# vqdang/hover_net

Hardware: NVIDIA B200
Metric: tiles/sec (higher is better)
Workload: dtype f16x3-split (fp32-equivalent products, fp32 accumulate); post-proc int32/f64

## Files before the change

### hover_net_b200/csrc/api.cu

```cuda
#include <cstring>
#include <memory>
#include <string>

#include "../../include/hvn.h"
#include "cnn.h"
#include "postproc.h"
#include "tile.h"

using namespace hvn;

static thread_local std::string g_err;

struct hvn_ctx {
    int device = 0;
    cudaStream_t stream = nullptr;
    std::unique_ptr<Model> model;
    Arena pp_arena;
    Arena io_arena;
    Arena tile_arena;
    int chunk = 0;
    int profile = 0;
    cudaEvent_t ev[4] = {nullptr, nullptr, nullptr, nullptr};
    cudaEvent_t tev[2] = {nullptr, nullptr};
    float ms_cnn = 0.f, ms_pp = 0.f;
// ... 94 lines not shown
    HVN_CHECK(c->model, HVN_ERR_STATE, "context has no model");
    c->model->finalize();
    API_END
}

int hvn_set_option(hvn_ctx *c, const char *key, int64_t value) {
    API_BEGIN
    use(c);
    std::string k = key ? key : "";
    if (k == "conv_path") { HVN_CHECK(c->model, HVN_ERR_STATE, "context has no model"); c->model->conv_path = (int)value; }
    else if (k == "chunk") c->chunk = (int)value;
    else if (k == "flood_impl") postproc_set_flood_impl((int)value);
    else if (k == "fuse_up2") { HVN_CHECK(c->model, HVN_ERR_STATE, "context has no model"); c->model->fuse_up2 = (int)value; }
    else if (k == "fuse_shortcut") { HVN_CHECK(c->model, HVN_ERR_STATE, "context has no model"); c->model->fuse_shortcut = (int)value; }
    else if (k == "stem_tc") { HVN_CHECK(c->model, HVN_ERR_STATE, "context has no model"); c->model->stem_tc = (int)value; }
    else if (k == "xform") { HVN_CHECK(c->model, HVN_ERR_STATE, "context has no model"); c->model->xform = (int)value; }
    else if (k == "branch_streams") { HVN_CHECK(c->model, HVN_ERR_STATE, "context has no model"); c->model->branch_streams = (int)value; }
    else if (k == "tc_seg_chunks") tc_set_seg_chunks((int)value);
    else if (k == "tc_block_n") tc_set_block_n((int)value);
    else if (k == "tc_res_tma") tc_set_res_tma((int)value);
    else if (k == "tc_xf_trunc") tc_set_xf_trunc((int)value);
    else if (k == "tc_ar") tc_set_ar((int)value);
    else if (k == "tc_lean_epi") tc_set_lean_epi((int)value);
    else if (k == "tc_rowstack") tc_set_rowstack((int)value);
    else if (k == "tc_xf_early") tc_set_xf_early((int)value);
    else if (k == "tc_prefetch") tc_set_prefetch((int)value);
    else if (k == "tc_ar_min_chunks") tc_set_ar_min_chunks((int)value);
    else if (k == "tc_ar_nres") tc_set_ar_nres((int)value);
    else if (k == "tc_ar_min_wst") tc_set_ar_min_wst((int)value);
    else if (k == "tc_res_tma_max_chunks") tc_set_res_tma_max_chunks((int)value);
// ... 411 lines not shown
```

### hover_net_b200/csrc/cnn.cu

```cuda
#include "cnn.h"

#include <algorithm>
#include <cmath>
#include <cstring>

namespace hvn {

static const struct { const char *name; int cin, c1, c3, units, stride; } kGroups[4] = {
    {"d0", 64, 64, 256, 3, 1}, {"d1", 256, 128, 512, 4, 2}, {"d2", 512, 256, 1024, 6, 2}, {"d3", 1024, 512, 2048, 3, 2}};

Plan::~Plan() {
    for (void *p : allocs) cudaFree(p);
}

template <typename T> T *Model::dalloc(size_t n, std::vector<void *> &owner, bool zero) {
    T *p = nullptr;
    HVN_CUDA(cudaMalloc((void **)&p, std::max<size_t>(n, 1) * sizeof(T)));
    owner.push_back(p);
    if (zero) HVN_CUDA(cudaMemset(p, 0, std::max<size_t>(n, 1) * sizeof(T)));
    return p;
}

void Model::add_spec(const std::string &name, std::initializer_list<int64_t> shape, bool ignored) {
    ParamSpec s;
// ... 393 lines not shown
    v.hi += off; v.lo += off; v.h = h; v.w = w; v.c = c;
    return v;
}
RawRef rview(const RawRef &b, int y0, int x0, int h, int w, int c0, int c) {
    RawRef v = b;
    v.p += (long long)y0 * b.sH + (long long)x0 * b.sW + c0;
    v.h = h; v.w = w; v.c = c;
    return v;
}
}

Plan &Model::plan(int B, int H, int W) {
    HVN_CHECK(finalized, -5, "weights not finalised (call hvn_finalize_weights)");
    HVN_CHECK(H == W, -1, "only square patches are supported (reference patch geometry is square)");
    std::string key = std::to_string(B) + "x" + std::to_string(H) + "x" + std::to_string(W) + "p" + std::to_string(conv_path) +
                      "b" + std::to_string(branch_streams) + "x" + std::to_string(xform) + "f" + std::to_string(fuse_shortcut) + "u" + std::to_string(fuse_up2) + "h" + std::to_string(tc_halo);
    auto it = plans_.find(key);
    if (it != plans_.end()) return *it->second;
    std::unique_ptr<Plan> pl(new Plan());
    Plan &P = *pl;
    P.B = B; P.H = H; P.W = W;
    out_shape(H, W, P.oh, P.ow, P.oc);

    auto new_split = [&](int h, int w, int c) {
        SplitRef r;
        size_t n = (size_t)B * h * w * c;
        r.hi = dalloc<__half>(n, P.allocs, true);
        r.lo = dalloc<__half>(n, P.allocs, true);
        P.bytes += 2 * n * sizeof(__half);
        r.sN = (long long)h * w * c; r.sH = w * c; r.sW = c; r.h = h; r.w = w; r.c = c;
        r.flag = d_flag_;
// ... 56 lines not shown
        op.c0_out = X0; op.c0_pad = mode == "fast" ? 3 : 0;
        op.bn = bn_.at("conv0.bn");
        op.flops = 2.0 * B * s0 * s0 * 64 * 147;
        P.ops.push_back(op);
    }
    SplitRef x = X0, D[4];
    int si = s0, ds[4];
    for (int gi = 0; gi < 4; ++gi) {
        const auto &g = kGroups[gi];
        const std::string gn = g.name;
        int so = (si + g.stride - 1) / g.stride;
        RawRef S = new_raw(so, so, g.c3);
        SplitRef A1 = new_split(si, si, g.c1), A2 = new_split(so, so, g.c1), Pp = new_split(so, so, g.c3);
        const bool fuse = fuse_shortcut != 0;
        if (!fuse) { Op &op = add_conv(gn + ".shortcut.weight", x, g.stride, 0, so, so); op.cp.out_raw = S; }
        for (int u = 0; u < g.units; ++u) {
            std::string p = gn + ".units." + std::to_string(u) + ".";
            const SplitRef &in = u == 0 ? x : Pp;
            int ri = u == 0 ? si : so, st = u == 0 ? g.stride : 1;
            SplitRef a1 = A1;
            if (ri != A1.h) { a1.h = ri; a1.w = ri; a1.sH = ri * g.c1; a1.sN = (long long)ri * ri * g.c1; }
            {
                Op &op = add_conv(p + "conv1.weight", in, 1, 0, ri, ri);
                set_bn(op, p + "conv1/bn", a1);
                if (u != 0 && use_xf) {
                    const BNParams &pb = bn_.at(p + "preact/bn");
                    op.cp.a_raw = S; op.cp.in_scale = pb.scale; op.cp.in_shift = pb.shift;
                }
            }
            int lo = tf_same_lo(ri, 3, st);
            { Op &op = add_conv(p + "conv2.weight", a1, st, lo, so, so); set_bn(op, p + "conv2/bn", A2); }
            {
                Op &op = add_conv(p + "conv3.weight", A2, 1, 0, so, so);
                if (u == 0 && fuse) {
                    op.cp.w = conv_.at(gn + ".fused3");
                    op.cp.a2 = x; op.cp.a2_stride = g.stride; op.cp.cin1 = g.c1;
                    op.flops += 2.0 * B * so * so * (double)g.cin * g.c3;
                    op.name = gn + ".units.0.conv3+shortcut";
                } else op.cp.res = S;
                if (u + 1 < g.units) {
                    op.cp.out_raw = S;
                    if (!use_xf) set_bn(op, gn + ".units." + std::to_string(u + 1) + ".preact/bn", Pp);
                } else set_bn(op, gn + ".blk_bna.bn", Pp);
            }
        }
        x = Pp; D[gi] = Pp; ds[gi] = so; si = so;
    }
    HVN_CHECK(2 * ds[3] == ds[2] && 2 * ds[2] == ds[1] && 2 * ds[1] == ds[0], -1, "patch size breaks the skip geometry");
    auto crop_to = [&](const SplitRef &d, int t) {
        int c = d.h - t;
        HVN_CHECK(c >= 0, -1, "skip connection smaller than decoder tensor");
        return sview(d, c / 2, c / 2, t, t, 0, d.c);
    };
    SplitRef U3in = new_split(2 * ds[3], 2 * ds[3], 1024);
    if (fuse_up2) {
        Op &op = add_conv("conv_bot.weight", D[3], 1, 0, ds[3], ds[3]);
        op.cp.up2 = 1; op.cp.skip = crop_to(D[2], 2 * ds[3]); op.cp.out_split = U3in;
    } else {
// ... 67 lines not shown
        if (b == 0) P.ops[first_op].fork_point = true;
        head.head.feat[b] = Hf[b];
        head.head.w[b] = head_w_.at(bp + "u0.conv");
        head.head.bias[b] = head_b_.at(bp + "u0.conv");
        head.head.out_ch[b] = branches_[b] == "tp" ? nr_types : 2;
        head.head.kind[b] = branches_[b] == "tp" ? HEAD_TP : (branches_[b] == "np" ? HEAD_NP : HEAD_HV);
        head.flops += 2.0 * B * ho * ho * 64 * head.head.out_ch[b];
    }
    cur_stream = 0;
    P.ops.push_back(head);

    tc_set_halo(tc_halo);
    for (auto &op : P.ops) {
        P.flops += op.flops;
        if (op.kind == Op::CONV && conv_path != 1) tc_plan(op.cp, op.tc);
    }
    plans_[key] = std::move(pl);
    return *plans_[key];
}

void Model::forward(const uint8_t *imgs, int B, int H, int W, float *out, int chunk, cudaStream_t s) {
    HVN_CHECK(finalized, -5, "weights not finalised (call hvn_finalize_weights)");
    HVN_CHECK(B >= 1, -1, "empty batch");
    int oh, ow, oc;
    out_shape(H, W, oh, ow, oc);
    if (chunk <= 0) chunk = 32;
    if (!side_[0]) {
        for (auto &st : side_) HVN_CUDA(cudaStreamCreateWithFlags(&st, cudaStreamNonBlocking));
        HVN_CUDA(cudaEventCreateWithFlags(&ev_fork_, cudaEventDisableTiming));
        for (auto &e : ev_join_) HVN_CUDA(cudaEventCreateWithFlags(&e, cudaEventDisableTiming));
// ... 43 lines not shown
                r.cls = "conv0";
                break;
            case Op::CONV:
                if (op.tc.ok && conv_path == 2) selftest_conv(op, s);
                if (op.tc.ok) { tc_launch(op.cp, op.tc, s); ++tc_launches; r.cls = "conv_tc"; }
                else {
                    ConvParams q = op.cp;
                    if (q.in_scale) {
                        launch_bnrelu(q.a_raw, bc, q.in_scale, q.in_shift, q.a, s);
                        q.in_scale = q.in_shift = nullptr;
                    }
                    launch_conv_ref(q, s);
                    r.cls = "conv_ref";
                }
                break;
            case Op::BNRELU:
                launch_bnrelu(op.bn_in, bc, op.bn.scale, op.bn.shift, op.bn_out, s);
                r.cls = "bnrelu";
                break;
            case Op::UP2ADD:
                launch_up2_add(op.up_in, bc, op.up_skip, op.up_out, s);
                r.cls = "bnrelu";
                break;
            case Op::HEAD: {
                HeadParams hp = op.head;
                hp.out = out + (size_t)b0 * oh * ow * oc;
                launch_head(hp, s);
                r.cls = "head";
                break;
            }
// ... 2 lines not shown
            if (profile_ops) { HVN_CUDA(cudaEventRecord(r.b, s)); recs.push_back(r); }
        }
    }
    s = main_stream;
    HVN_CUDA(cudaMemcpyAsync(h_flag_, d_flag_, sizeof(unsigned int), cudaMemcpyDeviceToHost, s));
    HVN_CUDA(cudaGetLastError());
    if (profile_ops) {
        HVN_CUDA(cudaStreamSynchronize(s));
        for (auto &r : recs) {
            float ms = 0.f;
            HVN_CUDA(cudaEventElapsedTime(&ms, r.a, r.b));
            class_ms[r.cls] += ms; class_flops[r.cls] += r.flops; class_launches[r.cls] += 1;
            if (profile_ops >= 2) {
                char line[384];
                const Op &o = *r.op;
                if (o.kind == Op::CONV)
                    snprintf(line, sizeof(line), "%-44s %-8s k%dx%d s%d cin%-4d cout%-4d out%dx%d box=%dx%d%s bn=%d %8.4f ms %8.2f GFLOP %7.1f TFLOP/s\n",
                             o.name.c_str(), r.cls, o.cp.w.kh, o.cp.w.kw, o.cp.stride, o.cp.w.cin, o.cp.w.cout, o.cp.ho, o.cp.wo,
                             o.tc.bw, o.tc.bh, o.tc.halo ? "H" : "", o.tc.block_n, ms, r.flops / 1e9, r.flops / 1e9 / std::max(ms, 1e-6f));
                else
                    snprintf(line, sizeof(line), "%-44s %-8s %8.4f ms\n", o.name.c_str(), r.cls, ms);
                debug_log += line;
            }
            cudaEventDestroy(r.a); cudaEventDestroy(r.b);
        }
    }
}

}
```

### hover_net_b200/csrc/cnn.h

```cpp
#pragma once
#include <map>
#include <memory>
#include <string>
#include <vector>

#include "cnn_kernels.h"
#include "common.cuh"

namespace hvn {

struct ParamSpec {
    std::string name;
    int ndim = 0;
    int64_t shape[4] = {0, 0, 0, 0};
    bool ignored = false;
    bool loaded = false;
    size_t numel() const {
        size_t n = 1;
        for (int i = 0; i < ndim; ++i) n *= (size_t)shape[i];
        return n;
    }
};

struct BNParams { float *scale = nullptr, *shift = nullptr; int c = 0; };

struct Op {
    enum Kind { CONV0, CONV, BNRELU, HEAD, UP2ADD } kind = CONV;
    std::string name;
    ConvParams cp;
    TcPlan tc;
    SplitRef c0_out; int c0_pad = 0;
    RawRef bn_in; SplitRef bn_out; BNParams bn;
    HeadParams head;
    RawRef up_in; SplitRef up_skip, up_out;
    double flops = 0;
    int stream = 0;
    bool fork_point = false;
};

struct Plan {
    int B = 0, H = 0, W = 0, oh = 0, ow = 0, oc = 0;
    std::vector<Op> ops;
    std::vector<void *> allocs;
    size_t bytes = 0;
    double flops = 0;
// ... 4 lines not shown
  public:
    Model(const std::string &mode, int nr_types);
    ~Model();
    std::string mode;
    int nr_types;
    int k;
    std::vector<ParamSpec> spec;
    std::map<std::string, int> index;
    std::map<std::string, std::vector<float>> host;
    bool finalized = false;
    int tc_halo = 1;
    int fuse_up2 = 0;
    int fuse_shortcut = 1;
    int stem_tc = 1;
    int xform = 1;
    int branch_streams = 1;
    int conv_path = 0;
    int act_shift = 0;
    bool range_overflow() const { return h_flag_ && *h_flag_ != 0; }
    void reset_range_flag(cudaStream_t s);

    void load(const std::string &name, const float *data, int ndim, const int64_t *shape);
    void finalize();
    void out_shape(int H, int W, int &oh, int &ow, int &oc) const;
    Plan &plan(int B, int H, int W);
    void forward(const uint8_t *imgs, int B, int H, int W, float *out, int chunk, cudaStream_t s);

    long long kernel_launches = 0, tc_launches = 0;
    int profile_ops = 0;
    std::map<std::string, double> class_ms, class_flops;
// ... 29 lines not shown
```

### hover_net_b200/csrc/cnn_kernels.h

```cpp
#pragma once
#include <cuda_runtime.h>
#include "conv_params.h"

#define HVN_MAX_TYPES 16

namespace hvn {

enum HeadKind { HEAD_TP = 0, HEAD_NP = 1, HEAD_HV = 2 };

struct HeadParams {
    int nbranch = 0;
    SplitRef feat[3];
    const float *w[3] = {nullptr, nullptr, nullptr};
    const float *bias[3] = {nullptr, nullptr, nullptr};
    int out_ch[3] = {0, 0, 0};
    int kind[3] = {0, 0, 0};
    int B = 0, h = 0, w_ = 0, C = 0;
    float *out = nullptr;
};

void launch_conv_ref(const ConvParams &P, cudaStream_t s);
void launch_conv0(const uint8_t *img, int B, int H, int W, int pad, const float *wgt, const float *scale,
                  const float *shift, const SplitRef &out, cudaStream_t s);
bool conv0_tc_supported(int H, int W, int pad, const SplitRef &out);
// ... 9 lines not shown
    unsigned char tmap_a_hi[128], tmap_a_lo[128], tmap_w_hi[128], tmap_w_lo[128];
    unsigned char tmap_a2_hi[128], tmap_a2_lo[128];
    int bw = 0, bh = 0;
    int tiles_x = 0, tiles_y = 0;
    int block_n = 0;
    int flat = 0;
    int res_tma = 0;
    int rs = 0, rs_bw = 0, rs_bh = 0;
    unsigned char tmap_rs_w_hi[128], tmap_rs_w_lo[128];
    int ar = 0, ar_gn = 1;
    int halo = 0;
    int halo_w = 0, halo_h = 0;
};
bool tc_plan(const ConvParams &P, TcPlan &plan);
void tc_launch(const ConvParams &P, const TcPlan &plan, cudaStream_t s);
void tc_set_block_n(int n);
void tc_set_seg_chunks(int n);
void tc_set_res_tma(int on);
void tc_set_res_tma_max_chunks(int n);
void tc_set_ar(int on);
void tc_set_ar_min_chunks(int n);
void tc_set_ar_nres(int n);
void tc_set_ar_min_wst(int n);
void tc_set_prefetch(int n);
void tc_set_rowstack(int on);
void tc_set_lean_epi(int on);
void tc_set_xf_early(int on);
void tc_set_xf_trunc(int on);
void tc_set_halo(int mode);

// ... 2 lines not shown
```

### hover_net_b200/csrc/conv_tc.cu

```cuda
#include <cuda.h>
#include <cuda_runtime.h>

#include <mutex>

#include "common.cuh"
#include "conv_epilogue.cuh"
#include "cnn_kernels.h"

namespace hvn {

__device__ __forceinline__ uint32_t smem_u32(const void *p) { return (uint32_t)__cvta_generic_to_shared(p); }

__device__ __forceinline__ void mbar_init(uint32_t bar, uint32_t count) {
    asm volatile("mbarrier.init.shared::cta.b64 [%0], %1;" ::"r"(bar), "r"(count) : "memory");
}
__device__ __forceinline__ void mbar_expect_tx(uint32_t bar, uint32_t bytes) {
    asm volatile("mbarrier.arrive.expect_tx.shared::cta.b64 _, [%0], %1;" ::"r"(bar), "r"(bytes) : "memory");
}
__device__ __forceinline__ void mbar_arrive(uint32_t bar) {
    asm volatile("mbarrier.arrive.shared::cta.b64 _, [%0];" ::"r"(bar) : "memory");
}
__device__ __forceinline__ void mbar_wait(uint32_t bar, uint32_t parity) {
    uint32_t ok;
    do {
// ... 28 lines not shown
    asm volatile(
        "{\n\t.reg .pred p;\n\t"
        "setp.ne.b32 p, %4, 0;\n\t"
        "tcgen05.mma.cta_group::1.kind::f16 [%0], %1, %2, %3, p;\n\t}"
        ::"r"(tmem_d), "l"(adesc), "l"(bdesc), "r"(idesc), "r"(accum) : "memory");
}
__device__ __forceinline__ void tc_ld32(uint32_t taddr, uint32_t (&r)[32]) {
    asm volatile(
        "tcgen05.ld.sync.aligned.32x32b.x32.b32 "
        "{%0, %1, %2, %3, %4, %5, %6, %7, %8, %9, %10, %11, %12, %13, %14, %15, "
        "%16, %17, %18, %19, %20, %21, %22, %23, %24, %25, %26, %27, %28, %29, %30, %31}, [%32];"
        : "=r"(r[0]), "=r"(r[1]), "=r"(r[2]), "=r"(r[3]), "=r"(r[4]), "=r"(r[5]), "=r"(r[6]), "=r"(r[7]),
          "=r"(r[8]), "=r"(r[9]), "=r"(r[10]), "=r"(r[11]), "=r"(r[12]), "=r"(r[13]), "=r"(r[14]), "=r"(r[15]),
          "=r"(r[16]), "=r"(r[17]), "=r"(r[18]), "=r"(r[19]), "=r"(r[20]), "=r"(r[21]), "=r"(r[22]), "=r"(r[23]),
          "=r"(r[24]), "=r"(r[25]), "=r"(r[26]), "=r"(r[27]), "=r"(r[28]), "=r"(r[29]), "=r"(r[30]), "=r"(r[31])
        : "r"(taddr) : "memory");
}
__device__ __forceinline__ void tc_ld_wait() { asm volatile("tcgen05.wait::ld.sync.aligned;" ::: "memory"); }

__device__ __forceinline__ uint64_t umma_desc(uint32_t saddr, uint32_t sbo = 1024) {
    uint64_t d = 0;
    d |= (uint64_t)((saddr & 0x3FFFFu) >> 4);
    d |= (uint64_t)1 << 16;
    d |= (uint64_t)(sbo >> 4) << 32;
    d |= (uint64_t)1 << 46;
    d |= (uint64_t)2 << 61;
    return d;
}

struct TcGeom {
// ... 726 lines not shown
                }
                asm volatile("fence.proxy.async.shared::cta;" ::: "memory");
                __syncwarp();
                if (lane == 0) request_res(tc + G.nres);
            }
        }
    }
    tc_fence_before();
    __syncthreads();
    if (warp == 1) {
        tc_fence_after();
        asm volatile("tcgen05.dealloc.cta_group::1.sync.aligned.b32 %0, %1;" ::"r"(tmem_base), "r"(TMEM_COLS) : "memory");
    }
}

struct RsGeom {
    int bw, bh, rows, tiles_y, tiles_m, kchunks, kh, seg;
};
template <int KW> constexpr int rs_stages() { return KW >= 5 ? 2 : 3; }
template <int KW> constexpr int rs_max_rows() { return KW >= 5 ? 124 : 128; }
template <int KW> constexpr int rs_stage_bytes() { return 2 * A_TILE_BYTES + 2 * KW * 32 * 128; }
template <int KW> constexpr int rs_smem() {
    return 1024 + rs_stages<KW>() * rs_stage_bytes<KW>() + 2 * rs_max_rows<KW>() * (KW * 16 + 4) * 4 + 8 * (2 * rs_stages<KW>() + 4) + 16;
}

__device__ __forceinline__ void tc_ld16(uint32_t taddr, uint32_t (&r)[16]) {
    asm volatile(
        "tcgen05.ld.sync.aligned.32x32b.x16.b32 "
        "{%0, %1, %2, %3, %4, %5, %6, %7, %8, %9, %10, %11, %12, %13, %14, %15}, [%16];"
        : "=r"(r[0]), "=r"(r[1]), "=r"(r[2]), "=r"(r[3]), "=r"(r[4]), "=r"(r[5]), "=r"(r[6]), "=r"(r[7]),
          "=r"(r[8]), "=r"(r[9]), "=r"(r[10]), "=r"(r[11]), "=r"(r[12]), "=r"(r[13]), "=r"(r[14]), "=r"(r[15])
        : "r"(taddr) : "memory");
}

template <int KW>
__global__ void __launch_bounds__(TC_THREADS, 1)
k_conv_rs(const __grid_constant__ CUtensorMap tm_a_hi, const __grid_constant__ CUtensorMap tm_a_lo,
          const __grid_constant__ CUtensorMap tm_w_hi, const __grid_constant__ CUtensorMap tm_w_lo,
          const ConvParams P, const RsGeom G) {
    constexpr int N = KW * 32, STAGES = rs_stages<KW>(), STAGE_BYTES = rs_stage_bytes<KW>();
    constexpr int W_PLANE = N * 128;
    constexpr int NH = KW * 16, STRIDE = NH + 4;
    extern __shared__ __align__(1024) uint8_t smem_raw[];
    const uint32_t smem_base = (smem_u32(smem_raw) + 1023u) & ~1023u;
    const uint32_t st_base = smem_base + STAGES * STAGE_BYTES;
    const uint32_t bar_base = st_base + 2u * rs_max_rows<KW>() * STRIDE * 4u;
    auto full_bar = [&](int s) { return bar_base + 8u * s; };
// ... 702 lines not shown
    }
    static int sms = 0;
    if (!sms) {
        int dev = 0;
        cudaGetDevice(&dev);
        cudaDeviceGetAttribute(&sms, cudaDevAttrMultiProcessorCount, dev);
    }
    const int grid = std::min(G.tiles_m * G.ngroups, sms);
    CUtensorMap a_hi, a_lo, w_hi, w_lo, res;
    memcpy(&a_hi, plan.tmap_a_hi, 128); memcpy(&a_lo, plan.tmap_a_lo, 128);
    memcpy(&w_hi, plan.tmap_w_hi, 128); memcpy(&w_lo, plan.tmap_w_lo, 128);
    memcpy(&res, plan.tmap_a2_lo, 128);
    k_conv_ar<<<grid, TC_THREADS, smem, s>>>(a_hi, a_lo, w_hi, w_lo, res, P, G);
}

template <int KW>
static void launch_rs(const ConvParams &P, const TcPlan &plan, cudaStream_t s) {
    RsGeom G;
    G.bw = plan.rs_bw; G.bh = plan.rs_bh; G.rows = G.bw * G.bh;
    G.tiles_y = cdiv(P.ho, G.bh); G.tiles_m = P.B * G.tiles_y;
    G.kchunks = P.w.cin_pad / 64; G.kh = P.w.kh; G.seg = g_seg_chunks;
    constexpr int smem = rs_smem<KW>();
    static_assert(smem <= SMEM_LIMIT, "conv_rs: shared memory budget exceeded");
    static bool attr = false;
    if (!attr) {
        HVN_CUDA(cudaFuncSetAttribute(k_conv_rs<KW>, cudaFuncAttributeMaxDynamicSharedMemorySize, smem));
        attr = true;
    }
    static int sms = 0;
    if (!sms) {
// ... 49 lines not shown
```

Measured before the change: 697.9.

## Fuse d0 conv3 with next unit's conv1 in a single tcgen05 kernel

Adds a persistent tcgen05 kernel that computes a d0 unit's 1x1 conv3 (256 outputs, raw residual output) and then, from the same tile, the next unit's preact BN+ReLU and 1x1 conv1 (64 outputs) with its BN+ReLU, written as a hi/lo split. This removes a separate conv1 launch and the re-read of the 256-channel activation from global memory for the d0 group. It costs a more complex warp-specialised pipeline with a second TMEM accumulator and doubled epilogue warps. Enabled by default via fuse_d0=1, which skips unit 0.

```diff
diff --git a/hover_net_b200/csrc/api.cu b/hover_net_b200/csrc/api.cu
--- a/hover_net_b200/csrc/api.cu
+++ b/hover_net_b200/csrc/api.cu
@@ -132,6 +132,7 @@
     else if (k == "fuse_up2") { HVN_CHECK(c->model, HVN_ERR_STATE, "context has no model"); c->model->fuse_up2 = (int)value; }
     else if (k == "fuse_shortcut") { HVN_CHECK(c->model, HVN_ERR_STATE, "context has no model"); c->model->fuse_shortcut = (int)value; }
     else if (k == "stem_tc") { HVN_CHECK(c->model, HVN_ERR_STATE, "context has no model"); c->model->stem_tc = (int)value; }
+    else if (k == "fuse_d0") { HVN_CHECK(c->model, HVN_ERR_STATE, "context has no model"); c->model->fuse_d0 = (int)value; }
     else if (k == "xform") { HVN_CHECK(c->model, HVN_ERR_STATE, "context has no model"); c->model->xform = (int)value; }
     else if (k == "branch_streams") { HVN_CHECK(c->model, HVN_ERR_STATE, "context has no model"); c->model->branch_streams = (int)value; }
     else if (k == "tc_seg_chunks") tc_set_seg_chunks((int)value);
diff --git a/hover_net_b200/csrc/cnn.cu b/hover_net_b200/csrc/cnn.cu
--- a/hover_net_b200/csrc/cnn.cu
+++ b/hover_net_b200/csrc/cnn.cu
@@ -431,7 +431,8 @@
     HVN_CHECK(finalized, -5, "weights not finalised (call hvn_finalize_weights)");
     HVN_CHECK(H == W, -1, "only square patches are supported (reference patch geometry is square)");
     std::string key = std::to_string(B) + "x" + std::to_string(H) + "x" + std::to_string(W) + "p" + std::to_string(conv_path) +
-                      "b" + std::to_string(branch_streams) + "x" + std::to_string(xform) + "f" + std::to_string(fuse_shortcut) + "u" + std::to_string(fuse_up2) + "h" + std::to_string(tc_halo);
+                      "b" + std::to_string(branch_streams) + "x" + std::to_string(xform) + "f" + std::to_string(fuse_shortcut) + "u" + std::to_string(fuse_up2) + "h" + std::to_string(tc_halo) +
+                      "d" + std::to_string(fuse_d0);
     auto it = plans_.find(key);
     if (it != plans_.end()) return *it->second;
     std::unique_ptr<Plan> pl(new Plan());
@@ -518,13 +519,15 @@
         SplitRef A1 = new_split(si, si, g.c1), A2 = new_split(so, so, g.c1), Pp = new_split(so, so, g.c3);
         const bool fuse = fuse_shortcut != 0;
         if (!fuse) { Op &op = add_conv(gn + ".shortcut.weight", x, g.stride, 0, so, so); op.cp.out_raw = S; }
+        const bool fuse_c1 = fuse_d0 && use_xf && conv_path == 0 && g.c1 == 64 && g.c3 == 256 && g.stride == 1;
+        bool conv1_fused = false;
         for (int u = 0; u < g.units; ++u) {
             std::string p = gn + ".units." + std::to_string(u) + ".";
             const SplitRef &in = u == 0 ? x : Pp;
             int ri = u == 0 ? si : so, st = u == 0 ? g.stride : 1;
             SplitRef a1 = A1;
             if (ri != A1.h) { a1.h = ri; a1.w = ri; a1.sH = ri * g.c1; a1.sN = (long long)ri * ri * g.c1; }
-            {
+            if (!conv1_fused) {
                 Op &op = add_conv(p + "conv1.weight", in, 1, 0, ri, ri);
                 set_bn(op, p + "conv1/bn", a1);
                 if (u != 0 && use_xf) {
@@ -546,6 +549,18 @@
                     op.cp.out_raw = S;
                     if (!use_xf) set_bn(op, gn + ".units." + std::to_string(u + 1) + ".preact/bn", Pp);
                 } else set_bn(op, gn + ".blk_bna.bn", Pp);
+                conv1_fused = fuse_c1 && u + 1 < g.units && (u >= 1 || fuse_d0 >= 2);
+                if (conv1_fused) {
+                    const std::string q = gn + ".units." + std::to_string(u + 1) + ".";
+                    const BNParams &pb = bn_.at(q + "preact/bn"), &b1 = bn_.at(q + "conv1/bn");
+                    op.kind = Op::CONV_C1;
+                    op.name += "+" + q + "conv1";
+                    op.c1.w = conv_.at(q + "conv1.weight");
+                    op.c1.in_scale = pb.scale; op.c1.in_shift = pb.shift;
+                    op.c1.scale = b1.scale; op.c1.shift = b1.shift;
+                    op.c1.out = A1;
+                    op.flops += 2.0 * B * so * so * (double)spec[index.at(q + "conv1.weight")].numel();
+                }
             }
         }
         x = Pp; D[gi] = Pp; ds[gi] = so; si = so;
@@ -643,6 +658,8 @@
     for (auto &op : P.ops) {
         P.flops += op.flops;
         if (op.kind == Op::CONV && conv_path != 1) tc_plan(op.cp, op.tc);
+        if (op.kind == Op::CONV_C1)
+            HVN_CHECK(tc_plan_c1(op.cp, op.c1, op.tc1), -1, "conv_ar_c1: layer " + op.name + " not supported (set fuse_d0=0)");
     }
     plans_[key] = std::move(pl);
     return *plans_[key];
@@ -716,6 +733,11 @@
                     r.cls = "conv_ref";
                 }
                 break;
+            case Op::CONV_C1:
+                tc_launch_c1(op.cp, op.c1, op.tc1, s);
+                ++tc_launches;
+                r.cls = "conv_tc";
+                break;
             case Op::BNRELU:
                 launch_bnrelu(op.bn_in, bc, op.bn.scale, op.bn.shift, op.bn_out, s);
                 r.cls = "bnrelu";
@@ -748,9 +770,9 @@
             if (profile_ops >= 2) {
                 char line[384];
                 const Op &o = *r.op;
-                if (o.kind == Op::CONV)
+                if (o.kind == Op::CONV || o.kind == Op::CONV_C1)
                     snprintf(line, sizeof(line), "%-44s %-8s k%dx%d s%d cin%-4d cout%-4d out%dx%d box=%dx%d%s bn=%d %8.4f ms %8.2f GFLOP %7.1f TFLOP/s\n",
-                             o.name.c_str(), r.cls, o.cp.w.kh, o.cp.w.kw, o.cp.stride, o.cp.w.cin, o.cp.w.cout, o.cp.ho, o.cp.wo,
+                             o.name.c_str(), o.kind == Op::CONV_C1 ? "conv_c1" : r.cls, o.cp.w.kh, o.cp.w.kw, o.cp.stride, o.cp.w.cin, o.cp.w.cout, o.cp.ho, o.cp.wo,
                              o.tc.bw, o.tc.bh, o.tc.halo ? "H" : "", o.tc.block_n, ms, r.flops / 1e9, r.flops / 1e9 / std::max(ms, 1e-6f));
                 else
                     snprintf(line, sizeof(line), "%-44s %-8s %8.4f ms\n", o.name.c_str(), r.cls, ms);
diff --git a/hover_net_b200/csrc/cnn.h b/hover_net_b200/csrc/cnn.h
--- a/hover_net_b200/csrc/cnn.h
+++ b/hover_net_b200/csrc/cnn.h
@@ -25,10 +25,12 @@
 struct BNParams { float *scale = nullptr, *shift = nullptr; int c = 0; };
 
 struct Op {
-    enum Kind { CONV0, CONV, BNRELU, HEAD, UP2ADD } kind = CONV;
+    enum Kind { CONV0, CONV, BNRELU, HEAD, UP2ADD, CONV_C1 } kind = CONV;
     std::string name;
     ConvParams cp;
     TcPlan tc;
+    C1Params c1;
+    TcC1Plan tc1;
     SplitRef c0_out; int c0_pad = 0;
     RawRef bn_in; SplitRef bn_out; BNParams bn;
     HeadParams head;
@@ -63,6 +65,7 @@
     int fuse_shortcut = 1;
     int stem_tc = 1;
     int xform = 1;
+    int fuse_d0 = 1;
     int branch_streams = 1;
     int conv_path = 0;
     int act_shift = 0;
diff --git a/hover_net_b200/csrc/cnn_kernels.h b/hover_net_b200/csrc/cnn_kernels.h
--- a/hover_net_b200/csrc/cnn_kernels.h
+++ b/hover_net_b200/csrc/cnn_kernels.h
@@ -47,6 +47,21 @@
 };
 bool tc_plan(const ConvParams &P, TcPlan &plan);
 void tc_launch(const ConvParams &P, const TcPlan &plan, cudaStream_t s);
+
+struct C1Params {
+    ConvWeights w;
+    const float *in_scale = nullptr, *in_shift = nullptr;
+    const float *scale = nullptr, *shift = nullptr;
+    SplitRef out;
+};
+struct TcC1Plan {
+    bool ok = false;
+    unsigned char tmap_a_hi[128], tmap_a_lo[128], tmap_a2_hi[128], tmap_a2_lo[128];
+    unsigned char tmap_w_hi[128], tmap_w_lo[128], tmap_w1_hi[128], tmap_w1_lo[128];
+    unsigned char tmap_res[128];
+};
+bool tc_plan_c1(const ConvParams &P, const C1Params &C, TcC1Plan &plan);
+void tc_launch_c1(const ConvParams &P, const C1Params &C, const TcC1Plan &plan, cudaStream_t s);
 void tc_set_block_n(int n);
 void tc_set_seg_chunks(int n);
 void tc_set_res_tma(int on);
diff --git a/hover_net_b200/csrc/conv_tc.cu b/hover_net_b200/csrc/conv_tc.cu
--- a/hover_net_b200/csrc/conv_tc.cu
+++ b/hover_net_b200/csrc/conv_tc.cu
@@ -66,6 +66,14 @@
           "=r"(r[8]), "=r"(r[9]), "=r"(r[10]), "=r"(r[11]), "=r"(r[12]), "=r"(r[13]), "=r"(r[14]), "=r"(r[15]),
           "=r"(r[16]), "=r"(r[17]), "=r"(r[18]), "=r"(r[19]), "=r"(r[20]), "=r"(r[21]), "=r"(r[22]), "=r"(r[23]),
           "=r"(r[24]), "=r"(r[25]), "=r"(r[26]), "=r"(r[27]), "=r"(r[28]), "=r"(r[29]), "=r"(r[30]), "=r"(r[31])
+        : "r"(taddr) : "memory");
+}
+__device__ __forceinline__ void tc_ld16(uint32_t taddr, uint32_t (&r)[16]) {
+    asm volatile(
+        "tcgen05.ld.sync.aligned.32x32b.x16.b32 "
+        "{%0, %1, %2, %3, %4, %5, %6, %7, %8, %9, %10, %11, %12, %13, %14, %15}, [%16];"
+        : "=r"(r[0]), "=r"(r[1]), "=r"(r[2]), "=r"(r[3]), "=r"(r[4]), "=r"(r[5]), "=r"(r[6]), "=r"(r[7]),
+          "=r"(r[8]), "=r"(r[9]), "=r"(r[10]), "=r"(r[11]), "=r"(r[12]), "=r"(r[13]), "=r"(r[14]), "=r"(r[15])
         : "r"(taddr) : "memory");
 }
 __device__ __forceinline__ void tc_ld_wait() { asm volatile("tcgen05.wait::ld.sync.aligned;" ::: "memory"); }
@@ -822,6 +830,308 @@
     }
 }
 
+struct C1Geom {
+    int tiles_m, kchunks, k1, wst, nres, has_res, pf, trunc;
+    long long m_total;
+};
+constexpr int C1_MAX_K = 2, C1_N1 = 64;
+constexpr int C1_EP_WARPS = 2 * EP_WARPS;
+constexpr int C1_THREADS = 64 + C1_EP_WARPS * 32;
+
+__global__ void __launch_bounds__(C1_THREADS, 1)
+k_conv_ar_c1(const __grid_constant__ CUtensorMap tm_a_hi, const __grid_constant__ CUtensorMap tm_a_lo,
+             const __grid_constant__ CUtensorMap tm_a2_hi, const __grid_constant__ CUtensorMap tm_a2_lo,
+             const __grid_constant__ CUtensorMap tm_w_hi, const __grid_constant__ CUtensorMap tm_w_lo,
+             const __grid_constant__ CUtensorMap tm_w1_hi, const __grid_constant__ CUtensorMap tm_w1_lo,
+             const __grid_constant__ CUtensorMap tm_res, const ConvParams P, const C1Params C, const C1Geom G) {
+    extern __shared__ __align__(1024) uint8_t smem_raw[];
+    const uint32_t smem_base = (smem_u32(smem_raw) + 1023u) & ~1023u;
+    const uint32_t x_base = smem_base + (uint32_t)G.kchunks * AR_A_SLICE;
+    const uint32_t w_base = x_base + 2u * AR_A_SLICE;
+    const uint32_t r_base = w_base + (uint32_t)G.wst * AR_W_STAGE;
+    const uint32_t bar_base = r_base + (uint32_t)G.nres * C1_EP_WARPS * 4096u;
+    auto afull_bar = [&](int k) { return bar_base + 8u * k; };
+    auto aempty_bar = [&](int k) { return bar_base + 8u * (C1_MAX_K + k); };
+    auto xfull_bar = [&](int x) { return bar_base + 8u * (2 * C1_MAX_K + x); };
+    auto xempty_bar = [&](int x) { return bar_base + 8u * (2 * C1_MAX_K + 2 + x); };
+    auto tfull_bar = [&](int s) { return bar_base + 8u * (2 * C1_MAX_K + 4 + s); };
+    auto tempty_bar = [&](int s) { return bar_base + 8u * (2 * C1_MAX_K + 6 + s); };
+    auto t1full_bar = [&](int s) { return bar_base + 8u * (2 * C1_MAX_K + 8 + s); };
+    auto t1empty_bar = [&](int s) { return bar_base + 8u * (2 * C1_MAX_K + 10 + s); };
+    auto wfull_bar = [&](int s) { return bar_base + 8u * (2 * C1_MAX_K + 12 + s); };
+    auto wempty_bar = [&](int s) { return bar_base + 8u * (2 * C1_MAX_K + 12 + AR_MAX_WST + s); };
+    auto rfull_bar = [&](int w, int r) { return bar_base + 8u * (2 * C1_MAX_K + 12 + 2 * AR_MAX_WST + AR_MAX_NRES * w + r); };
+    const uint32_t tmem_slot = bar_base + 8u * (2 * C1_MAX_K + 12 + 2 * AR_MAX_WST + AR_MAX_NRES * C1_EP_WARPS);
+    volatile uint32_t *tmem_slot_ptr = reinterpret_cast<volatile uint32_t *>(smem_raw + (tmem_slot - smem_u32(smem_raw)));
+    const int warp = threadIdx.x >> 5, lane = threadIdx.x & 31;
+    constexpr uint32_t TMEM_COLS = 512;
+    constexpr uint32_t T1_COL = 4 * AR_BN;
+    constexpr uint32_t kSeq = 0x76352410u;
+
+    if (warp == 0 && lane == 0) {
+        for (int k = 0; k < C1_MAX_K; ++k) { mbar_init(afull_bar(k), 1); mbar_init(aempty_bar(k), 1); }
+        for (int x = 0; x < 2; ++x) { mbar_init(xfull_bar(x), EP_WARPS); mbar_init(xempty_bar(x), 1); }
+        for (int s = 0; s < 2; ++s) {
+            mbar_init(tfull_bar(s), 1); mbar_init(tempty_bar(s), EP_WARPS * 32);
+            mbar_init(t1full_bar(s), 1); mbar_init(t1empty_bar(s), EP_WARPS * 32);
+        }
+        for (int s = 0; s < AR_MAX_WST; ++s) { mbar_init(wfull_bar(s), 1); mbar_init(wempty_bar(s), 1); }
+        for (int w = 0; w < C1_EP_WARPS; ++w)
+            for (int r = 0; r < AR_MAX_NRES; ++r) mbar_init(rfull_bar(w, r), 1);
+        asm volatile("fence.mbarrier_init.release.cluster;" ::: "memory");
+    }
+    if (warp == 1) {
+        asm volatile("tcgen05.alloc.cta_group::1.sync.aligned.shared::cta.b32 [%0], %1;" ::"r"(tmem_slot), "r"(TMEM_COLS) : "memory");
+        asm volatile("tcgen05.relinquish_alloc_permit.cta_group::1.sync.aligned;" ::: "memory");
+    }
+    tc_fence_before();
+    __syncthreads();
+    tc_fence_after();
+    const uint32_t tmem_base = *tmem_slot_ptr;
+    const int units = G.tiles_m;
+
+    if (warp == 0) {
+        if (lane == 0) {
+            int uc = 0, wit = 0;
+            auto load_w = [&](const CUtensorMap *hi, const CUtensorMap *lo, int c0, int c1) {
+                const int s = wit % G.wst;
+                mbar_wait(wempty_bar(s), (((uint32_t)(wit / G.wst)) & 1u) ^ 1u);
+                mbar_expect_tx(wfull_bar(s), (uint32_t)AR_W_STAGE);
+                const uint32_t b = w_base + (uint32_t)s * AR_W_STAGE;
+                tma_3d(b, hi, wfull_bar(s), c0, c1, 0);
+                tma_3d(b + AR_BN * 128, lo, wfull_bar(s), c0, c1, 0);
+                ++wit;
+            };
+            for (int u = blockIdx.x; u < units; u += gridDim.x, ++uc) {
+                const int m0 = u * 128;
+                if (G.pf > 0 && u + (int)gridDim.x < units) {
+                    const int m0n = (u + (int)gridDim.x) * 128;
+                    for (int kc = 0; kc < G.kchunks; ++kc) {
+                        const CUtensorMap *mh = kc < G.k1 ? &tm_a_hi : &tm_a2_hi, *ml = kc < G.k1 ? &tm_a_lo : &tm_a2_lo;
+                        const int c = (kc < G.k1 ? kc : kc - G.k1) * 64;
+                        tma_prefetch_2d(mh, c, m0n); tma_prefetch_2d(ml, c, m0n);
+                    }
+                }
+#pragma unroll 1
+                for (int st = 0; st < 8; ++st) {
+                    const int op = (int)((kSeq >> (4 * st)) & 15u);
+                    if (op >= 4) { load_w(&tm_w1_hi, &tm_w1_lo, (op - 4) * 64, 0); continue; }
+                    for (int kc = 0; kc < G.kchunks; ++kc) {
+                        if (op == 0) {
+                            mbar_wait(aempty_bar(kc), ((uint32_t)uc & 1u) ^ 1u);
+                            mbar_expect_tx(afull_bar(kc), (uint32_t)AR_A_SLICE);
+                            const uint32_t a = smem_base + (uint32_t)kc * AR_A_SLICE;
+                            if (kc < G.k1) {
+                                tma_2d(a, &tm_a_hi, afull_bar(kc), kc * 64, m0);
+                                tma_2d(a + A_TILE_BYTES, &tm_a_lo, afull_bar(kc), kc * 64, m0);
+                            } else {
+                                tma_2d(a, &tm_a2_hi, afull_bar(kc), (kc - G.k1) * 64, m0);
+                                tma_2d(a + A_TILE_BYTES, &tm_a2_lo, afull_bar(kc), (kc - G.k1) * 64, m0);
+                            }
+                        }
+                        load_w(&tm_w_hi, &tm_w_lo, kc * 64, op * AR_BN);
+                    }
+                }
+            }
+        }
+    } else if (warp == 1) {
+        if (lane == 0) {
+            const uint32_t idesc = (1u << 4) | ((uint32_t)(AR_BN >> 3) << 17) | ((uint32_t)(128 >> 4) << 24);
+            const uint32_t idesc2 = (1u << 4) | ((uint32_t)(2 * AR_BN >> 3) << 17) | ((uint32_t)(128 >> 4) << 24);
+            int uc = 0, wit = 0, tc = 0, xc = 0;
+            auto mma_slice = [&](uint32_t d_tmem, uint32_t sa, bool first) {
+                const int s = wit % G.wst;
+                mbar_wait(wfull_bar(s), ((uint32_t)(wit / G.wst)) & 1u);
+                tc_fence_after();
+                const uint64_t da_hi = umma_desc(sa), da_lo = umma_desc(sa + A_TILE_BYTES),
+                               db_hi = umma_desc(w_base + (uint32_t)s * AR_W_STAGE);
+#pragma unroll
+                for (int k = 0; k < 4; ++k) {
+                    const uint64_t ko = (uint64_t)(2 * k);
+                    tc_mma_f16(d_tmem, da_hi + ko, db_hi + ko, idesc2, (!first || k > 0) ? 1u : 0u);
+                    tc_mma_f16(d_tmem, da_lo + ko, db_hi + ko, idesc, 1u);
+                }
+                tc_commit(wempty_bar(s));
+                ++wit;
+            };
+            for (int u = blockIdx.x; u < units; u += gridDim.x, ++uc) {
+#pragma unroll 1
+                for (int st = 0; st < 8; ++st) {
+                    const int op = (int)((kSeq >> (4 * st)) & 15u);
+                    if (op < 4) {
+                        const int as = tc & 1;
+                        mbar_wait(tempty_bar(as), (((uint32_t)(tc >> 1)) & 1u) ^ 1u);
+                        tc_fence_after();
+                        for (int kc = 0; kc < G.kchunks; ++kc) {
+                            if (op == 0) mbar_wait(afull_bar(kc), (uint32_t)uc & 1u);
+                            mma_slice(tmem_base + (uint32_t)(as * 2 * AR_BN), smem_base + (uint32_t)kc * AR_A_SLICE, kc == 0);
+                            if (op == 3) tc_commit(aempty_bar(kc));
+                        }
+                        tc_commit(tfull_bar(as));
+                        ++tc;
+                    } else {
+                        const int j = op - 4, b1 = uc & 1;
+                        if (j == 0) {
+                            mbar_wait(t1empty_bar(b1), (((uint32_t)(uc >> 1)) & 1u) ^ 1u);
+                            tc_fence_after();
+                        }
+                        const int xs = xc & 1;
+                        mbar_wait(xfull_bar(xs), ((uint32_t)(xc >> 1)) & 1u);
+                        mma_slice(tmem_base + T1_COL + (uint32_t)(b1 * 2 * C1_N1), x_base + (uint32_t)xs * AR_A_SLICE, j == 0);
+                        tc_commit(xempty_bar(xs));
+                        ++xc;
+                        if (j == 3) tc_commit(t1full_bar(b1));
+                    }
+                }
+            }
+        }
+    } else {
+        const int ew = warp - 2, grp = ew >> 3, quad = warp & 3, half = (ew & 7) >> 2;
+        const uint32_t reg_addr0 = r_base + (uint32_t)(ew * G.nres) * 4096u;
+        const int sub_px = lane >> 3, sub_g = lane & 7;
+        uint8_t *xs_gen = smem_raw + (x_base - smem_u32(smem_raw));
+        auto box_of = [&](int tl, int &c0, int &c1) {
+            const int u = blockIdx.x + (tl >> 1) * (int)gridDim.x;
+            if (u >= units) return false;
+            c0 = (grp + 2 * (tl & 1)) * AR_BN + half * 32;
+            c1 = u * 128 + quad * 32;
+            return true;
+        };
+        auto request_res = [&](int tl) {
+            int c0, c1;
+            if (!G.has_res || !box_of(tl, c0, c1)) return;
+            const int r = tl % G.nres;
+            mbar_expect_tx(rfull_bar(ew, r), 4096u);
+            tma_2d(reg_addr0 + (uint32_t)r * 4096u, &tm_res, rfull_bar(ew, r), c0, c1);
+            if (G.pf > 0 && box_of(tl + 2, c0, c1)) tma_prefetch_2d(&tm_res, c0, c1);
+        };
+        if (lane == 0) for (int r = 0; r < G.nres; ++r) request_res(r);
+        float rmax = 0.f;
+        int tc = 0, uc = 0;
+        for (int u = blockIdx.x; u < units; u += gridDim.x, ++uc) {
+            const long long mrow0 = (long long)u * 128 + quad * 32;
+            for (int j = grp; j < 4; j += 2, ++tc) {
+                const int ch4 = j * AR_BN + half * 32 + sub_g * 4;
+                const float4 isc = *reinterpret_cast<const float4 *>(C.in_scale + ch4);
+                const float4 ish = *reinterpret_cast<const float4 *>(C.in_shift + ch4);
+                const int as = grp;
+                mbar_wait(tfull_bar(as), (uint32_t)tc & 1u);
+                tc_fence_after();
+                const uint32_t t_addr = tmem_base + ((uint32_t)(quad * 32) << 16) + (uint32_t)(as * 2 * AR_BN + half * 32);
+                const int rr = tc % G.nres;
+                uint8_t *reg = smem_raw + (reg_addr0 + (uint32_t)rr * 4096u - smem_u32(smem_raw));
+                if (G.has_res) mbar_wait(rfull_bar(ew, rr), ((uint32_t)(tc / G.nres)) & 1u);
+                const float *osc = P.w.oscale + j * AR_BN + half * 32;
+#pragma unroll
+                for (int hc = 0; hc < 2; ++hc) {
+                uint32_t r0[16], r1[16];
+                tc_ld16(t_addr + (uint32_t)(16 * hc), r0);
+                tc_ld16(t_addr + (uint32_t)(AR_BN + 16 * hc), r1);
+                tc_ld_wait();
+                if (hc == 1) {
+                    tc_fence_before();
+                    mbar_arrive(tempty_bar(as));
+                }
+#pragma unroll
+                for (int c = 4 * hc; c < 4 * hc + 4; ++c) {
+                    const float4 ws = __ldg(reinterpret_cast<const float4 *>(osc + 4 * c));
+                    float4 *p = reinterpret_cast<float4 *>(reg + lane * 128 + ((c ^ (lane & 7)) << 4));
+                    float4 v;
+                    if (G.has_res) {
+                        v = *p;
+                        v.x = fmaf(__uint_as_float(r0[4 * (c - 4 * hc)]) + __uint_as_float(r1[4 * (c - 4 * hc)]), ws.x, v.x);
+                        v.y = fmaf(__uint_as_float(r0[4 * (c - 4 * hc) + 1]) + __uint_as_float(r1[4 * (c - 4 * hc) + 1]), ws.y, v.y);
+                        v.z = fmaf(__uint_as_float(r0[4 * (c - 4 * hc) + 2]) + __uint_as_float(r1[4 * (c - 4 * hc) + 2]), ws.z, v.z);
+                        v.w = fmaf(__uint_as_float(r0[4 * (c - 4 * hc) + 3]) + __uint_as_float(r1[4 * (c - 4 * hc) + 3]), ws.w, v.w);
+                    } else {
+                        v.x = ((0.f + __uint_as_float(r0[4 * (c - 4 * hc)])) + __uint_as_float(r1[4 * (c - 4 * hc)])) * ws.x;
+                        v.y = ((0.f + __uint_as_float(r0[4 * (c - 4 * hc) + 1])) + __uint_as_float(r1[4 * (c - 4 * hc) + 1])) * ws.y;
+                        v.z = ((0.f + __uint_as_float(r0[4 * (c - 4 * hc) + 2])) + __uint_as_float(r1[4 * (c - 4 * hc) + 2])) * ws.z;
+                        v.w = ((0.f + __uint_as_float(r0[4 * (c - 4 * hc) + 3])) + __uint_as_float(r1[4 * (c - 4 * hc) + 3])) * ws.w;
+                    }
+                    *p = v;
+                }
+                }
+                __syncwarp();
+                const int xsl = grp;
+                mbar_wait(xempty_bar(xsl), ((uint32_t)tc & 1u) ^ 1u);
+                uint8_t *xa_hi = xs_gen + xsl * AR_A_SLICE, *xa_lo = xa_hi + A_TILE_BYTES;
+#pragma unroll
+                for (int it = 0; it < 8; ++it) {
+                    const int px = it * 4 + sub_px;
+                    const float4 t = *reinterpret_cast<const float4 *>(reg + px * 128 + ((sub_g ^ (px & 7)) << 4));
+                    const long long m = mrow0 + px;
+                    if (m < G.m_total) *reinterpret_cast<float4 *>(P.out_raw.p + m * P.out_raw.sW + ch4) = t;
+                    float y4[4] = {fmaf(t.x, isc.x, ish.x), fmaf(t.y, isc.y, ish.y), fmaf(t.z, isc.z, ish.z), fmaf(t.w, isc.w, ish.w)};
+                    rmax = fmaxf(fmaxf(rmax, fmaxf(y4[0], y4[1])), fmaxf(y4[2], y4[3]));
+                    uint2 oh, ol;
+                    if (G.trunc) split4_relu_trunc(y4, oh, ol);
+                    else {
+#pragma unroll
+                        for (int i = 0; i < 4; ++i) y4[i] = fmaxf(y4[i], 0.f);
+                        split4_f32<true>(y4, oh, ol);
+                    }
+                    const int row = quad * 32 + px, l16 = half * 8 + sub_g;
+                    const int off = row * 128 + ((((l16 >> 1) ^ (row & 7))) << 4) + (l16 & 1) * 8;
+                    *reinterpret_cast<uint2 *>(xa_hi + off) = oh;
+                    *reinterpret_cast<uint2 *>(xa_lo + off) = ol;
+                }
+                asm volatile("fence.proxy.async.shared::cta;" ::: "memory");
+                __syncwarp();
+                if (lane == 0) { mbar_arrive(xfull_bar(xsl)); request_res(tc + G.nres); }
+            }
+            if (grp == 0) continue;
+            const int b1 = uc & 1;
+            mbar_wait(t1full_bar(b1), ((uint32_t)(uc >> 1)) & 1u);
+            tc_fence_after();
+            const uint32_t t1 = tmem_base + ((uint32_t)(quad * 32) << 16) + T1_COL + (uint32_t)(b1 * 2 * C1_N1 + half * 32);
+            const long long m = mrow0 + lane;
+            __half *oh_p = C.out.hi + m * C.out.sW + half * 32, *ol_p = C.out.lo + m * C.out.sW + half * 32;
+#pragma unroll
+            for (int hc = 0; hc < 2; ++hc) {
+                uint32_t r0[16], r1[16];
+                tc_ld16(t1 + (uint32_t)(16 * hc), r0);
+                tc_ld16(t1 + (uint32_t)(C1_N1 + 16 * hc), r1);
+                tc_ld_wait();
+                if (hc == 1) {
+                    tc_fence_before();
+                    mbar_arrive(t1empty_bar(b1));
+                }
+                if (m < G.m_total)
+#pragma unroll
+                for (int c = 4 * hc; c < 4 * hc + 4; c += 2) {
+                    uint2 oh[2], ol[2];
+#pragma unroll
+                    for (int h = 0; h < 2; ++h) {
+                        const int cc = half * 32 + 4 * (c + h);
+                        const float4 ws = __ldg(reinterpret_cast<const float4 *>(C.w.oscale + cc));
+                        const float4 sc = __ldg(reinterpret_cast<const float4 *>(C.scale + cc));
+                        const float4 sh = __ldg(reinterpret_cast<const float4 *>(C.shift + cc));
+                        const int k = 4 * (c + h - 4 * hc);
+                        float v[4] = {((0.f + __uint_as_float(r0[k])) + __uint_as_float(r1[k])) * ws.x,
+                                      ((0.f + __uint_as_float(r0[k + 1])) + __uint_as_float(r1[k + 1])) * ws.y,
+                                      ((0.f + __uint_as_float(r0[k + 2])) + __uint_as_float(r1[k + 2])) * ws.z,
+                                      ((0.f + __uint_as_float(r0[k + 3])) + __uint_as_float(r1[k + 3])) * ws.w};
+                        v[0] = v[0] * sc.x + sh.x; v[1] = v[1] * sc.y + sh.y; v[2] = v[2] * sc.z + sh.z; v[3] = v[3] * sc.w + sh.w;
+#pragma unroll
+                        for (int i = 0; i < 4; ++i) v[i] = fmaxf(v[i], 0.f);
+                        split4_f32(v, oh[h], ol[h], C.out.flag);
+                    }
+                    *reinterpret_cast<uint4 *>(oh_p + 4 * c) = make_uint4(oh[0].x, oh[0].y, oh[1].x, oh[1].y);
+                    *reinterpret_cast<uint4 *>(ol_p + 4 * c) = make_uint4(ol[0].x, ol[0].y, ol[1].x, ol[1].y);
+                }
+            }
+        }
+        if (rmax > 65504.f && C.out.flag) *C.out.flag = 1u;
+    }
+    tc_fence_before();
+    __syncthreads();
+    if (warp == 1) {
+        tc_fence_after();
+        asm volatile("tcgen05.dealloc.cta_group::1.sync.aligned.b32 %0, %1;" ::"r"(tmem_base), "r"(TMEM_COLS) : "memory");
+    }
+}
+
 struct RsGeom {
     int bw, bh, rows, tiles_y, tiles_m, kchunks, kh, seg;
 };
@@ -830,15 +1140,6 @@
 template <int KW> constexpr int rs_stage_bytes() { return 2 * A_TILE_BYTES + 2 * KW * 32 * 128; }
 template <int KW> constexpr int rs_smem() {
     return 1024 + rs_stages<KW>() * rs_stage_bytes<KW>() + 2 * rs_max_rows<KW>() * (KW * 16 + 4) * 4 + 8 * (2 * rs_stages<KW>() + 4) + 16;
-}
-
-__device__ __forceinline__ void tc_ld16(uint32_t taddr, uint32_t (&r)[16]) {
-    asm volatile(
-        "tcgen05.ld.sync.aligned.32x32b.x16.b32 "
-        "{%0, %1, %2, %3, %4, %5, %6, %7, %8, %9, %10, %11, %12, %13, %14, %15}, [%16];"
-        : "=r"(r[0]), "=r"(r[1]), "=r"(r[2]), "=r"(r[3]), "=r"(r[4]), "=r"(r[5]), "=r"(r[6]), "=r"(r[7]),
-          "=r"(r[8]), "=r"(r[9]), "=r"(r[10]), "=r"(r[11]), "=r"(r[12]), "=r"(r[13]), "=r"(r[14]), "=r"(r[15])
-        : "r"(taddr) : "memory");
 }
 
 template <int KW>
@@ -1571,6 +1872,104 @@
     k_conv_ar<<<grid, TC_THREADS, smem, s>>>(a_hi, a_lo, w_hi, w_lo, res, P, G);
 }
 
+bool tc_plan_c1(const ConvParams &P, const C1Params &C, TcC1Plan &plan) {
+    plan.ok = false;
+    const ConvWeights &w = P.w, &w1 = C.w;
+    const long long M = (long long)P.B * P.ho * P.wo;
+    if (w.taps != 1 || w.cout != 4 * AR_BN || w.cin_pad % 64 || w.cin_pad / 64 > C1_MAX_K || P.stride != 1 || P.pad_t || P.pad_l) return false;
+    if (w1.taps != 1 || w1.cout != C1_N1 || w1.cin_pad != w.cout || w1.cin != w.cout) return false;
+    if (P.in_scale || P.up2 || P.out_split.hi || !P.out_raw.p || !C.in_scale || !C.scale || !C.out.hi) return false;
+    if (M >= (1ll << 31) - 256) return false;
+    const bool two = P.a2.hi != nullptr;
+    if (two == (P.res.p != nullptr)) return false;
+    if (two && (P.cin1 % 64 || P.a2_stride != 1 || P.cin1 + P.a2.c != w.cin_pad)) return false;
+    if (!two && w.cin_pad != P.a.c) return false;
+    auto dense = [&](long long sW, long long sH, long long sN, int h, int wd, int c) {
+        return sW == c && sW * wd == sH && sH * h == sN && h == P.ho && wd == P.wo;
+    };
+    auto al = [](const void *p) { return !(reinterpret_cast<uintptr_t>(p) & 15); };
+    if (!dense(P.a.sW, P.a.sH, P.a.sN, P.a.h, P.a.w, P.a.c) || !al(P.a.hi) || !al(P.a.lo)) return false;
+    if (two && (!dense(P.a2.sW, P.a2.sH, P.a2.sN, P.a2.h, P.a2.w, P.a2.c) || !al(P.a2.hi) || !al(P.a2.lo))) return false;
+    if (!dense(P.out_raw.sW, P.out_raw.sH, P.out_raw.sN, P.out_raw.h, P.out_raw.w, w.cout) || !al(P.out_raw.p)) return false;
+    if (P.res.p && (!dense(P.res.sW, P.res.sH, P.res.sN, P.res.h, P.res.w, w.cout) || !al(P.res.p))) return false;
+    if (!dense(C.out.sW, C.out.sH, C.out.sN, C.out.h, C.out.w, C1_N1) || !al(C.out.hi) || !al(C.out.lo)) return false;
+    cuuint32_t ones[3] = {1, 1, 1};
+    cuuint32_t box[2] = {64, 128};
+    {
+        cuuint64_t dims[2] = {(cuuint64_t)P.a.c, (cuuint64_t)M};
+        cuuint64_t str[1] = {(cuuint64_t)P.a.sW * 2};
+        if (!encode(plan.tmap_a_hi, P.a.hi, 2, dims, str, box, ones) || !encode(plan.tmap_a_lo, P.a.lo, 2, dims, str, box, ones)) return false;
+    }
+    if (two) {
+        cuuint64_t dims[2] = {(cuuint64_t)P.a2.c, (cuuint64_t)M};
+        cuuint64_t str[1] = {(cuuint64_t)P.a2.sW * 2};
+        if (!encode(plan.tmap_a2_hi, P.a2.hi, 2, dims, str, box, ones) || !encode(plan.tmap_a2_lo, P.a2.lo, 2, dims, str, box, ones)) return false;
+    } else {
+        memcpy(plan.tmap_a2_hi, plan.tmap_a_hi, 128); memcpy(plan.tmap_a2_lo, plan.tmap_a_lo, 128);
+    }
+    if (P.res.p) {
+        cuuint64_t dims[2] = {(cuuint64_t)w.cout, (cuuint64_t)M};
+        cuuint64_t str[1] = {(cuuint64_t)P.res.sW * 4};
+        cuuint32_t rbox[2] = {32, 32};
+        if (!encode(plan.tmap_res, P.res.p, 2, dims, str, rbox, ones, true, true)) return false;
+    } else memcpy(plan.tmap_res, plan.tmap_a_hi, 128);
+    cuuint32_t wbox[3] = {64, (cuuint32_t)AR_BN, 1};
+    {
+        cuuint64_t dims[3] = {(cuuint64_t)w.cin_pad, (cuuint64_t)w.cout, 1};
+        cuuint64_t str[2] = {(cuuint64_t)w.cin_pad * 2, (cuuint64_t)w.cin_pad * w.cout * 2};
+        if (!encode(plan.tmap_w_hi, w.hi, 3, dims, str, wbox, ones) || !encode(plan.tmap_w_lo, w.lo, 3, dims, str, wbox, ones)) return false;
+    }
+    {
+        cuuint64_t dims[3] = {(cuuint64_t)w1.cin_pad, (cuuint64_t)w1.cout, 1};
+        cuuint64_t str[2] = {(cuuint64_t)w1.cin_pad * 2, (cuuint64_t)w1.cin_pad * w1.cout * 2};
+        if (!encode(plan.tmap_w1_hi, w1.hi, 3, dims, str, wbox, ones) || !encode(plan.tmap_w1_lo, w1.lo, 3, dims, str, wbox, ones)) return false;
+    }
+    plan.ok = true;
+    return true;
+}
+
+constexpr int c1_fixed_smem(int kchunks) {
+    return 1024 + kchunks * AR_A_SLICE + 2 * AR_A_SLICE + 8 * (2 * C1_MAX_K + 12 + 2 * AR_MAX_WST + AR_MAX_NRES * C1_EP_WARPS) + 16;
+}
+static_assert(c1_fixed_smem(C1_MAX_K) + C1_EP_WARPS * 4096 + 2 * AR_W_STAGE <= SMEM_LIMIT, "conv_ar_c1: shared memory budget exceeded");
+
+void tc_launch_c1(const ConvParams &P, const C1Params &C, const TcC1Plan &plan, cudaStream_t s) {
+    HVN_CHECK(plan.ok, -1, "conv_ar_c1: layer not planned");
+    C1Geom G;
+    G.kchunks = P.w.cin_pad / 64;
+    G.k1 = P.a2.hi ? P.cin1 / 64 : G.kchunks;
+    G.m_total = (long long)P.B * P.ho * P.wo;
+    G.tiles_m = cdiv(G.m_total, 128);
+    G.has_res = P.res.p != nullptr;
+    G.pf = g_pf;
+    G.trunc = g_xf_trunc;
+    int fixed = c1_fixed_smem(G.kchunks) + C1_EP_WARPS * 4096;
+    G.nres = 1;
+    if (G.has_res)
+        while (G.nres < std::min(g_ar_nres, AR_MAX_NRES) && fixed + C1_EP_WARPS * 4096 + g_ar_min_wst * AR_W_STAGE <= SMEM_LIMIT) {
+            ++G.nres; fixed += C1_EP_WARPS * 4096;
+        }
+    G.wst = std::min(AR_MAX_WST, (SMEM_LIMIT - fixed) / AR_W_STAGE);
+    HVN_CHECK(G.wst >= 2, -1, "conv_ar_c1: weight ring does not fit shared memory");
+    const int smem = fixed + G.wst * AR_W_STAGE;
+    static int attr_smem = 0;
+    if (smem > attr_smem) {
+        HVN_CUDA(cudaFuncSetAttribute(k_conv_ar_c1, cudaFuncAttributeMaxDynamicSharedMemorySize, smem));
+        attr_smem = smem;
+    }
+    static int sms = 0;
+    if (!sms) {
+        int dev = 0;
+        cudaGetDevice(&dev);
+        cudaDeviceGetAttribute(&sms, cudaDevAttrMultiProcessorCount, dev);
+    }
+    CUtensorMap m[9];
+    const unsigned char *src[9] = {plan.tmap_a_hi, plan.tmap_a_lo, plan.tmap_a2_hi, plan.tmap_a2_lo, plan.tmap_w_hi,
+                                   plan.tmap_w_lo, plan.tmap_w1_hi, plan.tmap_w1_lo, plan.tmap_res};
+    for (int i = 0; i < 9; ++i) memcpy(&m[i], src[i], 128);
+    k_conv_ar_c1<<<std::min(G.tiles_m, sms), C1_THREADS, smem, s>>>(m[0], m[1], m[2], m[3], m[4], m[5], m[6], m[7], m[8], P, C, G);
+}
+
 template <int KW>
 static void launch_rs(const ConvParams &P, const TcPlan &plan, cudaStream_t s) {
     RsGeom G;
```

Result: no change. 702.6 (median of 6 runs) (+0.7%).
